# adityamwagh/SuperSLAM

Measured on AMD Instinct MI355X. Metric: stereo pairs/sec (SPx2+LG) at 1376x376, higher is better.
Workload: dtype f16; 1 GPU; configs[1]: SuperPoint x2 + select + gather + 1x LightGlue on 1376x376 stereo pairs; a step = 8 x 64 = 512 pairs per GPU resident in HBM (8 library calls of 64 pairs, different images per call), max_keypoints 600, seeded synthetic weights; pairs_per_call=64, max_keypoints=600, matches_last_call=1412, parallelism=replicated weights, pairs sharded over 1 rank(s), no data-path collective

## Files before the change

### superslam_amd/csrc/conv_pp.hip

```cpp
#include <cstdio>
#include <cstdlib>
#include <string>
#include <type_traits>
#include <vector>

#include "igemm.h"
#include "kernels.h"

#ifndef SSHIP_PP_EPI
#define SSHIP_PP_EPI -1
#endif
#ifndef SSHIP_PP_COLMAJOR
#define SSHIP_PP_COLMAJOR 1
#endif
#ifndef SSHIP_PP_EPI_LAST
#define SSHIP_PP_EPI_LAST 0
#endif
#ifndef SSHIP_PP_EPI_FUSED
#define SSHIP_PP_EPI_FUSED 0
#endif
#ifndef SSHIP_PP_TRACE_BUILD
#define SSHIP_PP_TRACE_BUILD 0
#endif
#ifndef SSHIP_PP_PRIO
#define SSHIP_PP_PRIO 2
#endif
#ifndef SSHIP_PP_NBUF
#define SSHIP_PP_NBUF 3
#endif
#ifndef SSHIP_PP_ABL
#define SSHIP_PP_ABL 0
#endif
#ifndef SSHIP_PP_ACC_PRELOAD
#define SSHIP_PP_ACC_PRELOAD 1
#endif

namespace sship {

struct PpArgs {
  const _Float16* in;
  const uint8_t* img;
  const _Float16* w1a;
  const float* b1a;
  const _Float16* wpack;
  const float* bias;
  _Float16* out;
  int B, H, W, cout;
  unsigned long long* trace;
};

constexpr int P_TH = 8, P_TW = 32, P_THH = 10, P_TWH = 34;
constexpr int P_IN_HALFS = P_THH * P_TWH * 64;
constexpr int P_W_HALFS = 36864;
constexpr int P_IN_UNITS = P_THH * P_TWH * 8;
constexpr int P_IN_IT = (P_IN_UNITS + 255) / 256;
constexpr int P_NT1A = (P_THH * P_TWH + 31) / 32;

__device__ __forceinline__ int pp_lds(int row, int col, int unit) {
  return (row * P_TWH + col) * 64 + ((unit ^ ((col >> 1) & 7)) << 3);
}

struct PpWalk { int tx, ty, b; };

template <int CIN, int CT, bool POOL, bool FUSE1A>
__global__ __launch_bounds__(512, 2) void conv3x3_pp(PpArgs p) {
  constexpr int MT = CT / 32, NCHUNK = CIN / 64;
  constexpr int EPI_MFMA = FUSE1A ? SSHIP_PP_EPI_FUSED : SSHIP_PP_EPI < 0 ? (CIN == 128 ? 2 * MT : 0) : (SSHIP_PP_EPI > 2 * MT ? 2 * MT : SSHIP_PP_EPI);
  constexpr int PIX_B = CIN * 2;
  constexpr int NBUF = SSHIP_PP_NBUF;
  static_assert(NCHUNK * 9 * 4 * MT * 512 == P_W_HALFS, "weights must fill exactly 72 KiB");
  static_assert(!FUSE1A || CIN == 64, "conv1a fusion feeds a 64-channel layer");
  extern __shared__ __attribute__((aligned(16))) char smem[];
  _Float16* s_w = reinterpret_cast<_Float16*>(smem);
  const int tid = threadIdx.x, wave = tid >> 6, lane = tid & 63, j = lane & 31, hh = lane >> 5;
  const int grp = __builtin_amdgcn_readfirstlane(wave >> 2);
  const int gw = wave & 3, gt = tid & 255;
  _Float16* my_in = s_w + P_W_HALFS + grp * P_IN_HALFS;

  const int tiles_x = (p.W + P_TW - 1) / P_TW, tiles_y = (p.H + P_TH - 1) / P_TH;
  const int ntiles = p.B * tiles_x * tiles_y;
  const int cb = blockIdx.y;
  const int t_begin = (int)((long long)blockIdx.x * ntiles / gridDim.x);
  const int t_end = (int)((long long)(blockIdx.x + 1) * ntiles / gridDim.x);
  const int n_wg = t_end - t_begin;
  if (n_wg <= 0) return;
  const int T0 = (n_wg + 1) >> 1, T1 = n_wg >> 1, T_mine = grp ? T1 : T0;

  {
    const _Float16* wsrc = p.wpack + (size_t)cb * P_W_HALFS;
    for (int u = tid; u < P_W_HALFS / 8; u += 512)
      *reinterpret_cast<uint4*>(s_w + u * 8) = *reinterpret_cast<const uint4*>(wsrc + u * 8);
  }
  float* s_bias = reinterpret_cast<float*>(s_w + P_W_HALFS + 2 * P_IN_HALFS);
  if (tid < 2 * CT) s_bias[tid] = p.bias[cb * CT + (tid % CT)];
  int boff[3][4];
#pragma unroll
  for (int kx = 0; kx < 3; ++kx)
#pragma unroll
    for (int ks = 0; ks < 4; ++ks) boff[kx][ks] = (j + kx) * 64 + (((2 * ks + hh) ^ (((j + kx) >> 1) & 7)) << 3);

  auto walk_init = [&](int t) __attribute__((always_inline)) {
    PpWalk w;
    if constexpr (SSHIP_PP_COLMAJOR != 0 && !FUSE1A) {
      w.ty = t % tiles_y;
      const int r = t / tiles_y;
      w.tx = r % tiles_x; w.b = r / tiles_x;
    } else {
      w.tx = t % tiles_x;
      const int r = t / tiles_x;
      w.ty = r % tiles_y; w.b = r / tiles_y;
    }
    return w;
  };
  auto walk_next = [&](PpWalk& w) __attribute__((always_inline)) {
    if constexpr (SSHIP_PP_COLMAJOR != 0 && !FUSE1A) {
      w.ty += 2;
      while (w.ty >= tiles_y) {
        w.ty -= tiles_y;
        if (++w.tx == tiles_x) { w.tx = 0; ++w.b; }
      }
    } else {
      w.tx += 2;
      while (w.tx >= tiles_x) {
        w.tx -= tiles_x;
        if (++w.ty == tiles_y) { w.ty = 0; ++w.b; }
      }
    }
  };
  PpWalk pw = walk_init(t_begin + grp), sw = pw, ew = pw;

  typedef unsigned u4_t __attribute__((ext_vector_type(4)));
  constexpr unsigned P_OOB = 0xfffffff0u;
  const unsigned ep_voff = POOL ? ((j & 1) ? P_OOB : (unsigned)(((j >> 1) * p.cout + hh * 8) * 2)) : (unsigned)((j * p.cout + hh * 8) * 2);
  constexpr int P_ROW_UNITS = P_TWH * 8;
  u4_t rin[FUSE1A ? 1 : 11];
  const int m_px = gt >> 3, m_part = gt & 7;
  const int r_row = gt >> 4, r_px = 32 + ((gt & 15) >> 3), r_part = gt & 7;
  const bool r_on = gt < 160;
  const unsigned voff_main = (unsigned)(m_px * PIX_B + m_part * 16);
  const unsigned voff_rem = r_on ? (unsigned)((r_row * p.W + r_px) * PIX_B + r_part * 16) : P_OOB;
  _Float16* lds_main = my_in + pp_lds(0, m_px, m_part);
  _Float16* lds_rem = my_in + pp_lds(r_on ? r_row : 0, r_px, r_part);
  const unsigned row_bytes = (unsigned)(p.W * PIX_B);
  auto prefetch_in = [&](int chunk) __attribute__((always_inline)) {
    if constexpr (!FUSE1A) {
      const int y0 = pw.ty * P_TH, x0 = pw.tx * P_TW;
      const char* img = reinterpret_cast<const char*>(p.in) + (size_t)pw.b * p.H * p.W * PIX_B - (size_t)(p.W + 1) * PIX_B;
      const __amdgpu_buffer_rsrc_t rsrc = __builtin_amdgcn_make_buffer_rsrc(const_cast<char*>(img), 0, (int)0x7ffffff0, 0x00020000);
      const unsigned soff = (unsigned)(y0 * p.W + x0) * (unsigned)PIX_B + (unsigned)chunk * 128u;
      const bool interior = y0 >= 1 && y0 + P_TH + 1 <= p.H && x0 >= 1 && x0 + P_TW + 1 <= p.W;
      if (interior) {
#pragma unroll
        for (int i = 0; i < 10; ++i) rin[i] = __builtin_amdgcn_raw_buffer_load_b128(rsrc, voff_main, soff + i * row_bytes, 0);
        rin[10] = __builtin_amdgcn_raw_buffer_load_b128(rsrc, voff_rem, soff, 0);
      } else {
        const int rlo = y0 == 0 ? 1 : 0, rhi = min(P_THH - 1, p.H - y0), clo = x0 == 0 ? 1 : 0, chi = min(P_TWH - 1, p.W - x0);
        const unsigned vm = (m_px >= clo && m_px <= chi) ? voff_main : P_OOB;
#pragma unroll
        for (int i = 0; i < 10; ++i)
          rin[i] = __builtin_amdgcn_raw_buffer_load_b128(rsrc, (i >= rlo && i <= rhi) ? vm : P_OOB, soff + i * row_bytes, 0);
        const bool r_ok = r_px >= clo && r_px <= chi && r_row >= rlo && r_row <= rhi;
        rin[10] = __builtin_amdgcn_raw_buffer_load_b128(rsrc, r_ok ? voff_rem : P_OOB, soff, 0);
      }
      if (chunk == NCHUNK - 1) walk_next(pw);
    }
  };
  auto stage_in = [&]() __attribute__((always_inline)) {
    if constexpr (!FUSE1A) {
#pragma unroll
      for (int i = 0; i < 10; ++i) *reinterpret_cast<u4_t*>(lds_main + i * (P_TWH * 64)) = rin[i];
      if (r_on) *reinterpret_cast<u4_t*>(lds_rem) = rin[10];
    }
  };
  constexpr int NT_W = 3;
  unsigned rp[FUSE1A ? NT_W : 1][3];
  int c1_pypx[FUSE1A ? NT_W : 1], c1_lds[FUSE1A ? NT_W : 1];
  const unsigned c1_selA = hh ? 0x06050402u : 0x04020100u, c1_selB = hh ? 0x0c0c0d0du : 0x0c0c0c05u;
  if constexpr (FUSE1A) {
#pragma unroll
    for (int k = 0; k < NT_W; ++k) {
      const int q = min((gw + 4 * k) * 32 + j, P_THH * P_TWH - 1);
      const int py = q / P_TWH, px = q - py * P_TWH;
      c1_pypx[k] = (py << 16) | px;
      c1_lds[k] = ((py * P_TWH + px) * 64 + hh * 4) | (((px >> 1) & 7) << 24);
    }
  }
  auto prefetch_u8 = [&]() __attribute__((always_inline)) {
    if constexpr (FUSE1A) {
      const int y0 = pw.ty * P_TH, x0 = pw.tx * P_TW;
      const uint8_t* im = p.img + (size_t)pw.b * p.H * p.W;
      walk_next(pw);
      const bool interior = y0 >= 2 && y0 + P_TH + 2 <= p.H && x0 >= 2 && x0 + P_TW + 2 + 3 <= p.W;
#pragma unroll
      for (int k = 0; k < NT_W; ++k) {
        const int py = c1_pypx[k] >> 16, px = c1_pypx[k] & 0xffff;
        if (interior) {
          const uint8_t* pp = im + (size_t)(y0 - 2 + py) * p.W + (x0 - 2 + px);
#pragma unroll
          for (int r = 0; r < 3; ++r) {
            unsigned v;
            __builtin_memcpy(&v, pp + (size_t)r * p.W, 4);
            rp[k][r] = v;
          }
        } else {
#pragma unroll
          for (int r = 0; r < 3; ++r) {
            const int cy = min(max(y0 - 2 + py + r, 0), p.H - 1), cx = min(max(x0 - 2 + px, 0), p.W - 4);
            unsigned v;
            __builtin_memcpy(&v, im + (size_t)cy * p.W + cx, 4);
            rp[k][r] = v;
          }
        }
      }
    }
  };
  h8_t a1a0, a1a1;
  if constexpr (FUSE1A) {
    a1a0 = *reinterpret_cast<const h8_t*>(p.w1a + lane * 8);
    a1a1 = *reinterpret_cast<const h8_t*>(p.w1a + 512 + lane * 8);
  }
  unsigned long long* trow = p.trace + ((size_t)(blockIdx.y * gridDim.x + blockIdx.x) * 2 + grp) * 10;
  auto stage_conv1a = [&](bool tr_stage) __attribute__((always_inline)) {
    if constexpr (FUSE1A) {
      unsigned long long ts0 = 0, ts1 = 0, ts2 = 0;
      if (SSHIP_PP_TRACE_BUILD && tr_stage) ts0 = __builtin_readcyclecounter();
      const int y0 = sw.ty * P_TH, x0 = sw.tx * P_TW;
      walk_next(sw);
      const bool interior = y0 >= 1 && y0 + P_TH + 1 <= p.H && x0 >= 1 && x0 + P_TW + 1 <= p.W;
      const bool patch_interior = y0 >= 2 && y0 + P_TH + 2 <= p.H && x0 >= 2 && x0 + P_TW + 2 + 3 <= p.W;
      h8_t bf[NT_W];
#pragma unroll
      for (int k = 0; k < NT_W; ++k) {
        if (!patch_interior) {
          const int py = c1_pypx[k] >> 16, px = c1_pypx[k] & 0xffff;
          const int gx = x0 - 2 + px;
          const int sh = gx - min(max(gx, 0), p.W - 4);
#pragma unroll
          for (int r = 0; r < 3; ++r) {
            const int gy = y0 - 2 + py + r;
            unsigned v = rp[k][r];
            v = sh < 0 ? (sh <= -4 ? 0u : v << (-8 * sh)) : (sh >= 4 ? 0u : v >> (8 * sh));
            rp[k][r] = (gy >= 0 && gy < p.H) ? v : 0u;
          }
        }
        const unsigned X = hh ? rp[k][2] : rp[k][1], Y = hh ? rp[k][1] : rp[k][0];
        const unsigned q4 = __builtin_amdgcn_perm(X, Y, c1_selA), q2 = __builtin_amdgcn_perm(X, X, c1_selB);
        auto cv8 = [](unsigned w, int byte) __attribute__((always_inline)) {
          float r;
          asm("v_mul_f32 %0, %1, %2" : "=v"(r) : "v"((float)((w >> (8 * byte)) & 0xffu)), "v"(1.0f / 255.0f));
          return (_Float16)r;
        };
        bf[k][0] = cv8(q4, 0); bf[k][1] = cv8(q4, 1); bf[k][2] = cv8(q4, 2); bf[k][3] = cv8(q4, 3);
        bf[k][4] = cv8(q2, 0); bf[k][5] = cv8(q2, 1); bf[k][6] = (_Float16)0.f; bf[k][7] = (_Float16)0.f;
      }
      if (SSHIP_PP_TRACE_BUILD && tr_stage) ts1 = __builtin_readcyclecounter();
      const f16x_t zero16 = {0.f, 0.f, 0.f, 0.f, 0.f, 0.f, 0.f, 0.f, 0.f, 0.f, 0.f, 0.f, 0.f, 0.f, 0.f, 0.f};
      f16x_t d0[NT_W], d1[NT_W];
#pragma unroll
      for (int k = 0; k < NT_W; ++k) {
        if (gw + 4 * k >= P_NT1A) continue;
        d0[k] = mfma32(a1a0, bf[k], zero16);
        d1[k] = mfma32(a1a1, bf[k], zero16);
      }
      if (SSHIP_PP_TRACE_BUILD && tr_stage) ts2 = __builtin_readcyclecounter();
#pragma unroll
      for (int k = 0; k < NT_W; ++k) {
        if (gw + 4 * k >= P_NT1A) continue;
        if ((gw + 4 * k) * 32 + j < P_THH * P_TWH) {
          bool inside = true;
          if (!interior) {
            const int gy = y0 - 1 + (c1_pypx[k] >> 16), gx = x0 - 1 + (c1_pypx[k] & 0xffff);
            inside = gy >= 0 && gy < p.H && gx >= 0 && gx < p.W;
          }
          const int base = c1_lds[k] & 0xffffff, swz = c1_lds[k] >> 24;
#pragma unroll
          for (int g = 0; g < 4; ++g) {
            const h4_t z4 = {(_Float16)0.f, (_Float16)0.f, (_Float16)0.f, (_Float16)0.f};
            h4_t o0 = __builtin_elementwise_max(to_h4(d0[k][4 * g], d0[k][4 * g + 1], d0[k][4 * g + 2], d0[k][4 * g + 3]), z4);
            h4_t o1 = __builtin_elementwise_max(to_h4(d1[k][4 * g], d1[k][4 * g + 1], d1[k][4 * g + 2], d1[k][4 * g + 3]), z4);
            if (!interior && !inside) { o0 = z4; o1 = z4; }
            const int u0 = (g ^ swz) << 3;
            *reinterpret_cast<h4_t*>(my_in + base + u0) = o0;
            *reinterpret_cast<h4_t*>(my_in + base + (u0 ^ 32)) = o1;
          }
        }
      }
      if (SSHIP_PP_TRACE_BUILD && tr_stage) { trow[6] = ts1 - ts0; trow[7] = ts2 - ts1; trow[8] = __builtin_readcyclecounter() - ts2; }
    }
  };

  f16x_t acc[MT][2];
  auto acc_init = [&]() __attribute__((always_inline)) {
#pragma unroll
    for (int m = 0; m < MT; ++m)
#pragma unroll
      for (int n = 0; n < 2; ++n)
#pragma unroll
        for (int g = 0; g < 4; ++g) {
          const float4 b4 = *reinterpret_cast<const float4*>(s_bias + n * CT + m * 32 + hh * 4 + g * 8);
          acc[m][n][4 * g + 0] = b4.x; acc[m][n][4 * g + 1] = b4.y; acc[m][n][4 * g + 2] = b4.z; acc[m][n][4 * g + 3] = b4.w;
        }
  };
  auto mfma_item = [&](auto chunk_c) __attribute__((always_inline)) {
    constexpr int chunk = decltype(chunk_c)::value;
    const _Float16* wc = s_w + chunk * (9 * 4 * MT * 512) + lane * 8;
    const _Float16* ib = my_in + (gw * 2) * P_TWH * 64;
    h8_t fa[NBUF][MT], fb[NBUF][2];
    auto load_frags = [&](int idx, int buf) __attribute__((always_inline)) {
      const int h32 = idx / 18, r18 = idx - 18 * h32, t6 = r18 / 3;
      const int ky = CIN == 128 ? r18 - 3 * t6 : (idx >> 2) / 3, kx = CIN == 128 ? t6 >> 1 : (idx >> 2) - 3 * ky;
      const int tap = ky * 3 + kx, ks = CIN == 128 ? 2 * h32 + (t6 & 1) : idx & 3;
#pragma unroll
      for (int m = 0; m < MT; ++m) fa[buf][m] = *reinterpret_cast<const h8_t*>(wc + ((tap * 4 + ks) * MT + m) * 512);
#pragma unroll
      for (int n = 0; n < 2; ++n) fb[buf][n] = *reinterpret_cast<const h8_t*>(ib + (n + ky) * P_TWH * 64 + boff[kx][ks]);
    };
    if constexpr (CIN == 64 && SSHIP_K_ROWSHARE != 0) {
      h8_t ra[3][MT], rbq[6];
      auto loads_for = [&](int t) __attribute__((always_inline)) {
        const int g = t / 3, ky = t - 3 * g, kx = g >> 2, ks = g & 3;
#pragma unroll
        for (int m = 0; m < MT; ++m) ra[t % 3][m] = *reinterpret_cast<const h8_t*>(wc + (((ky * 3 + kx) * 4 + ks) * MT + m) * 512);
        if (ky == 0) {
          rbq[(4 * g) % 6] = *reinterpret_cast<const h8_t*>(ib + boff[kx][ks]);
          rbq[(4 * g + 1) % 6] = *reinterpret_cast<const h8_t*>(ib + P_TWH * 64 + boff[kx][ks]);
        } else {
          rbq[(4 * g + ky + 1) % 6] = *reinterpret_cast<const h8_t*>(ib + (ky + 1) * P_TWH * 64 + boff[kx][ks]);
        }
      };
      loads_for(0); loads_for(1);
      if constexpr (chunk == 0 && !SSHIP_PP_ACC_PRELOAD) acc_init();
#pragma unroll
      for (int t = 0; t < 36; ++t) {
        if (t + 2 < 36 && !(SSHIP_PP_ABL & 1)) loads_for(t + 2);
        __builtin_amdgcn_sched_barrier(0);
        const int g = t / 3, ky = t - 3 * g;
#pragma unroll
        for (int n = 0; n < 2; ++n)
#pragma unroll
          for (int m = 0; m < MT; ++m) {
            if constexpr ((SSHIP_PP_ABL & 2) != 0) asm volatile("" :: "v"(ra[t % 3][m]), "v"(rbq[(4 * g + ky + n) % 6]));
            else acc[m][n] = mfma32(ra[t % 3][m], rbq[(4 * g + ky + n) % 6], acc[m][n]);
          }
        __builtin_amdgcn_sched_barrier(0);
      }
      return;
    }
#pragma unroll
    for (int i = 0; i < NBUF - 1; ++i) load_frags(i, i);
    if constexpr (chunk == 0 && !SSHIP_PP_ACC_PRELOAD) acc_init();
#pragma unroll
    for (int idx = 0; idx < 36; ++idx) {
      if (idx + NBUF - 1 < 36 && !(SSHIP_PP_ABL & 1)) load_frags(idx + NBUF - 1, (idx + NBUF - 1) % NBUF);
      __builtin_amdgcn_sched_barrier(0);
#pragma unroll
      for (int n = 0; n < 2; ++n)
#pragma unroll
        for (int m = 0; m < MT; ++m) {
          if constexpr ((SSHIP_PP_ABL & 2) != 0) asm volatile("" :: "v"(fa[idx % NBUF][m]), "v"(fb[idx % NBUF][n]));
          else acc[m][n] = mfma32(fa[idx % NBUF][m], fb[idx % NBUF][n], acc[m][n]);
        }
      __builtin_amdgcn_sched_barrier(0);
    }
  };
  auto epilogue = [&](int u_lo, int u_hi) __attribute__((always_inline)) {
    const int y0 = ew.ty * P_TH, x0 = ew.tx * P_TW, b = ew.b;
    if (u_hi == 2 * MT) walk_next(ew);
    const int yb = y0 + __builtin_amdgcn_readfirstlane(gw) * 2;
    const h2_t z2 = {(_Float16)0.f, (_Float16)0.f};
    auto relu2 = [&](float lo, float hi) __attribute__((always_inline)) -> unsigned {
      h2_t v = {(_Float16)lo, (_Float16)hi};
      v = __builtin_elementwise_max(v, z2);
      return *reinterpret_cast<const unsigned*>(&v);
    };
    auto pack2 = [](float lo, float hi) __attribute__((always_inline)) -> unsigned {
      const h2_t v = {(_Float16)lo, (_Float16)hi};
      return *reinterpret_cast<const unsigned*>(&v);
    };
    const int Ho = POOL ? p.H >> 1 : p.H, Wo = POOL ? p.W >> 1 : p.W;
    const __amdgpu_buffer_rsrc_t ro = __builtin_amdgcn_make_buffer_rsrc(
        reinterpret_cast<char*>(p.out) + (size_t)b * Ho * Wo * p.cout * 2, 0, (int)0x7ffffff0, 0x00020000);
    const int xo0 = POOL ? x0 >> 1 : x0;
    unsigned voff = ep_voff;
    if (xo0 + (POOL ? P_TW / 2 : P_TW) > Wo)
      voff = (xo0 + (POOL ? j >> 1 : j)) < Wo ? ep_voff : P_OOB;
    auto store_pair = [&](int row_off, int m, int g, unsigned a0, unsigned a1, unsigned b0, unsigned b1) __attribute__((always_inline)) {
      const auto r0 = __builtin_amdgcn_permlane32_swap(a0, b0, false, false);
      const auto r1 = __builtin_amdgcn_permlane32_swap(a1, b1, false, false);
      int so = (row_off + cb * CT + m * 32 + g * 8) * 2;
      asm volatile("" : "+s"(so));
      typedef unsigned st4_t __attribute__((ext_vector_type(4)));
      if constexpr ((SSHIP_PP_ABL & 4) != 0) { asm volatile("" :: "v"(r0[0]), "v"(r1[0]), "v"(r0[1]), "v"(r1[1])); return; }
      __builtin_amdgcn_raw_buffer_store_b128(st4_t{r0[0], r1[0], r0[1], r1[1]}, ro, voff, so, 0);
    };
    if constexpr (!POOL) {
      const int x = x0 + j;
#pragma unroll
      for (int n = 0; n < 2; ++n) {
        const int y = yb + n;
        const bool ok = y < p.H && x < p.W;
        _Float16* pix = p.out + ((size_t)(b * p.H + y) * p.W + x) * p.cout + cb * CT;
#pragma unroll
        for (int m = 0; m < MT; ++m)
#pragma unroll
          for (int g = 0; g < 4; g += 2) {
            if (2 * m + g / 2 < u_lo || 2 * m + g / 2 >= u_hi) continue;
            const f16x_t& a = acc[m][n];
            const auto r0 = __builtin_amdgcn_permlane32_swap(relu2(a[4 * g + 0], a[4 * g + 1]), relu2(a[4 * g + 4], a[4 * g + 5]), false, false);
            const auto r1 = __builtin_amdgcn_permlane32_swap(relu2(a[4 * g + 2], a[4 * g + 3]), relu2(a[4 * g + 6], a[4 * g + 7]), false, false);
            if constexpr ((SSHIP_PP_ABL & 4) != 0) { asm volatile("" :: "v"(r0[0]), "v"(r1[0]), "v"(r0[1]), "v"(r1[1])); continue; }
            if (ok) *reinterpret_cast<uint4*>(pix + m * 32 + (g + hh) * 8) = make_uint4(r0[0], r1[0], r0[1], r1[1]);
          }
      }
    } else {
      const int yo = yb >> 1;
      if (yo >= Ho) voff = P_OOB;
      const int pix = (yo * Wo + xo0) * p.cout;
      auto pool1 = [&](int m, int r) __attribute__((always_inline)) -> float {
        const float tt = fmaxf(fmaxf(acc[m][0][r], acc[m][1][r]), 0.f);
        const float nb = __int_as_float(__builtin_amdgcn_update_dpp(0, __float_as_int(tt), 0xB1, 0xF, 0xF, false));
        return fmaxf(tt, nb);
      };
#pragma unroll
      for (int m = 0; m < MT; ++m)
#pragma unroll
        for (int g = 0; g < 4; g += 2) {
          if (2 * m + g / 2 < u_lo || 2 * m + g / 2 >= u_hi) continue;
          store_pair(pix, m, g, pack2(pool1(m, 4 * g + 0), pool1(m, 4 * g + 1)), pack2(pool1(m, 4 * g + 2), pool1(m, 4 * g + 3)),
                     pack2(pool1(m, 4 * g + 4), pool1(m, 4 * g + 5)), pack2(pool1(m, 4 * g + 6), pool1(m, 4 * g + 7)));
        }
    }
  };

  const bool tr_lane = SSHIP_PP_TRACE_BUILD && p.trace && gw == 0 && lane == 0;
  unsigned long long t0 = 0, t1 = 0;
  auto data_role = [&](bool do_epi, bool do_stage, bool do_prefetch, int pf_chunk, bool init_acc, bool tr) __attribute__((always_inline)) {
    if (SSHIP_PP_PRIO) __builtin_amdgcn_s_setprio(SSHIP_PP_PRIO);
    if (tr) t0 = __builtin_readcyclecounter();
    if (!SSHIP_PP_EPI_LAST && do_epi && EPI_MFMA < 2 * MT) epilogue(EPI_MFMA, 2 * MT);
    if (tr) { t1 = __builtin_readcyclecounter(); trow[0] = t1 - t0; t0 = t1; }
    if (do_stage) { if constexpr (FUSE1A) stage_conv1a(tr); else stage_in(); }
    if (tr) { t1 = __builtin_readcyclecounter(); trow[1] = t1 - t0; t0 = t1; }
    if (do_prefetch) { if constexpr (FUSE1A) prefetch_u8(); else prefetch_in(pf_chunk); }
    if (SSHIP_PP_EPI_LAST && do_epi && EPI_MFMA < 2 * MT) epilogue(EPI_MFMA, 2 * MT);
    if (SSHIP_PP_ACC_PRELOAD && init_acc) acc_init();
    if (tr) { t1 = __builtin_readcyclecounter(); trow[2] = t1 - t0; t0 = t1; }
    __syncthreads();
    if (tr) trow[4] = __builtin_readcyclecounter() - t0;
    if (SSHIP_PP_PRIO) __builtin_amdgcn_s_setprio(0);
  };
  auto mfma_role = [&](auto chunk_c, bool tr) __attribute__((always_inline)) {
    constexpr int chunk = decltype(chunk_c)::value;
    if (tr) t0 = __builtin_readcyclecounter();
    mfma_item(chunk_c);
    if constexpr (chunk == NCHUNK - 1 && EPI_MFMA > 0) epilogue(0, EPI_MFMA);
    if (tr) { t1 = __builtin_readcyclecounter(); trow[3] = t1 - t0; t0 = t1; }
    __syncthreads();
    if (tr) trow[5] = __builtin_readcyclecounter() - t0;
  };
  const std::integral_constant<int, 0> c0{};
  const std::integral_constant<int, NCHUNK - 1> c_last{};
  const int nbar_mine = grp + 1 + 2 * NCHUNK * T_mine, nbar_all = max(1 + 2 * NCHUNK * T0, 2 + 2 * NCHUNK * T1);
  if (T_mine > 0) { if constexpr (FUSE1A) prefetch_u8(); else prefetch_in(0); }
  __syncthreads();
  if (grp == 1) __syncthreads();
  data_role(false, T_mine > 0, NCHUNK > 1 ? T_mine > 0 : T_mine > 1, NCHUNK > 1 ? 1 : 0, T_mine > 0, false);
#pragma unroll 1
  for (int it = 0; it < T_mine; ++it) {
    const bool more = it + 1 < T_mine, tr = tr_lane && it == 2;
    if constexpr (NCHUNK == 1) {
      mfma_role(c0, tr);
      data_role(true, more, it + 2 < T_mine, 0, more, tr);
    } else {
      mfma_role(c0, tr);
      data_role(false, true, more, 0, false, tr);
      mfma_role(c_last, false);
      data_role(true, more, more, 1, more, false);
    }
  }
#pragma unroll 1
  for (int k = nbar_mine; k < nbar_all; ++k) __syncthreads();
}

template <int CIN, int CT, bool POOL, bool FUSE1A>
static hipError_t launch_pp(const PpArgs& a_in, hipStream_t s) {
  PpArgs a = a_in;
  constexpr size_t smem = (size_t)(2 * P_IN_HALFS + P_W_HALFS) * 2 + 128 * 4;
  static_assert(smem <= 163840, "LDS budget");
  auto kern = conv3x3_pp<CIN, CT, POOL, FUSE1A>;
  static const hipError_t attr_rc = hipFuncSetAttribute(reinterpret_cast<const void*>(kern), hipFuncAttributeMaxDynamicSharedMemorySize, (int)smem);
  if (attr_rc != hipSuccess) return attr_rc;
  const int ncb = a.cout / CT;
  const int ntiles = a.B * ((a.W + P_TW - 1) / P_TW) * ((a.H + P_TH - 1) / P_TH);
  int gx = cu_count() / ncb;
  if (gx < 1) gx = 1;
  if (gx * 2 > ntiles) gx = (ntiles + 1) / 2;
  if (gx < 1) gx = 1;
  static const bool trace_on = SSHIP_PP_TRACE_BUILD && dev_env("SSHIP_PP_TRACE") != nullptr;
  static unsigned long long* tbuf = nullptr;
  if (trace_on) {
    if (!tbuf) (void)hipMalloc(&tbuf, 4096 * 2 * 10 * 8);
    (void)hipMemsetAsync(tbuf, 0, 4096 * 2 * 10 * 8, s);
    a.trace = tbuf;
  }
  hipLaunchKernelGGL(kern, dim3(gx, ncb), dim3(512), smem, s, a);
  if (trace_on) {
    std::vector<unsigned long long> h(4096 * 2 * 10);
    (void)hipStreamSynchronize(s);
    (void)hipMemcpy(h.data(), tbuf, h.size() * 8, hipMemcpyDeviceToHost);
    double sum[10] = {0}; long cnt = 0;
    for (int i = 0; i < gx * ncb * 2; ++i) {
      if (!h[i * 10 + 3]) continue;
      for (int k = 0; k < 10; ++k) sum[k] += (double)h[i * 10 + k];
      ++cnt;
    }
    if (cnt) fprintf(stderr, "[pp trace cin=%d ct=%d pool=%d fuse=%d] epilogue=%.0f stage=%.0f prefetch=%.0f | mfma=%.0f | barrier wait after data=%.0f after mfma=%.0f (clk, %ld groups)\n",
                     CIN, CT, (int)POOL, (int)FUSE1A, sum[0] / cnt, sum[1] / cnt, sum[2] / cnt, sum[3] / cnt, sum[4] / cnt, sum[5] / cnt, cnt);
    if (cnt && sum[6] > 0) fprintf(stderr, "[pp trace   conv1a staging] convert=%.0f mfma issue=%.0f relu+lds writes=%.0f clk\n", sum[6] / cnt, sum[7] / cnt, sum[8] / cnt);
  }
  return hipGetLastError();
}

hipError_t sp_conv3x3_pp(const ConvW& w, const _Float16* in, _Float16* out, int B, int H, int W, bool pool, hipStream_t s) {
  if ((size_t)H * W * w.cin * 2 >= 0x7f000000ull) return hipErrorInvalidValue;
  PpArgs a{};
  a.in = in; a.wpack = w.w; a.bias = w.bias; a.out = out; a.B = B; a.H = H; a.W = W; a.cout = w.cout;
  static const bool dma64 = [] { const char* e = dev_env("SUPERSLAM_HIP_CONV64"); return e && std::string(e) == "dma"; }();
  if (w.cin == 64 && w.w_q && dma64 && sp_conv3x3_pp128_fits(B, H, W, 64)) return sp_conv3x3_pp128(w, in, out, B, H, W, pool, s);
  if (w.cin == 64 && w.ct == 64) return pool ? launch_pp<64, 64, true, false>(a, s) : launch_pp<64, 64, false, false>(a, s);
  static const std::string c128 = [] { const char* e = dev_env("SUPERSLAM_HIP_CONV128"); return std::string(e ? e : ""); }();
  static const bool ct32 = c128 == "ct32";
  const int tiles16 = B * ((W + 31) / 32) * ((H + 15) / 16);
  const bool few_tiles = c128.empty() && w.ct == 32 && w.w && (tiles16 + 1) / 2 * (w.cout / 64) < cu_count();
  if (w.cin == 128 && w.w_q && !ct32 && !few_tiles && sp_conv3x3_pp128_fits(B, H, W, 128)) return sp_conv3x3_pp128(w, in, out, B, H, W, pool, s);
  if (w.cin == 128 && w.ct == 32) return pool ? launch_pp<128, 32, true, false>(a, s) : launch_pp<128, 32, false, false>(a, s);
  return hipErrorInvalidValue;
}

hipError_t sp_conv1ab_pp(const ConvW& w1b, const _Float16* w1a_frag, const float* b1a, const uint8_t* img, _Float16* out,
                         int B, int H, int W, hipStream_t s) {
  PpArgs a{};
  a.img = img; a.w1a = w1a_frag; a.b1a = b1a; a.wpack = w1b.w; a.bias = w1b.bias; a.out = out;
  a.B = B; a.H = H; a.W = W; a.cout = w1b.cout;
  if (w1b.cin != 64 || w1b.ct != 64) return hipErrorInvalidValue;
  return launch_pp<64, 64, true, true>(a, s);
}

}
```

Baseline: 5688 pairs/s.

## Keep conv1b weights in registers and repartition waves in fused conv1a+conv1b kernel

For the fused conv1a+conv1b (64-channel, pooled) kernel, each wave now holds its slice of the 3x3 weights in 36 VGPR fragments instead of reading them from a 72 KiB LDS copy. Waves split the two M-tiles by gw&1 and cover four output rows each, streaming input rows from LDS with a 6-deep rotating buffer. To free registers, the conv1a per-lane coordinate tables and weights move to LDS, and there is a new pooled epilogue path. This removes the LDS weight traffic and shrinks LDS use, but raises VGPR pressure and adds LDS lookups in the staging code.

After: 5693 pairs/s, median of 2. No clear change (+0.1%).

```diff
diff --git a/superslam_amd/csrc/conv_pp.hip b/superslam_amd/csrc/conv_pp.hip
--- a/superslam_amd/csrc/conv_pp.hip
+++ b/superslam_amd/csrc/conv_pp.hip
@@ -33,6 +33,9 @@
 #endif
 #ifndef SSHIP_PP_ACC_PRELOAD
 #define SSHIP_PP_ACC_PRELOAD 1
+#endif
+#ifndef SSHIP_PP_WREG
+#define SSHIP_PP_WREG 1
 #endif
 
 namespace sship {
@@ -55,6 +58,7 @@
 constexpr int P_IN_UNITS = P_THH * P_TWH * 8;
 constexpr int P_IN_IT = (P_IN_UNITS + 255) / 256;
 constexpr int P_NT1A = (P_THH * P_TWH + 31) / 32;
+constexpr bool pp_wreg(int cin, bool fuse1a) { return cin == 64 && fuse1a && SSHIP_PP_WREG != 0 && SSHIP_K_ROWSHARE != 0; }
 
 __device__ __forceinline__ int pp_lds(int row, int col, int unit) {
   return (row * P_TWH + col) * 64 + ((unit ^ ((col >> 1) & 7)) << 3);
@@ -67,15 +71,21 @@
   constexpr int MT = CT / 32, NCHUNK = CIN / 64;
   constexpr int EPI_MFMA = FUSE1A ? SSHIP_PP_EPI_FUSED : SSHIP_PP_EPI < 0 ? (CIN == 128 ? 2 * MT : 0) : (SSHIP_PP_EPI > 2 * MT ? 2 * MT : SSHIP_PP_EPI);
   constexpr int PIX_B = CIN * 2;
+  constexpr bool WREG = pp_wreg(CIN, FUSE1A);
+  constexpr int MW = WREG ? 1 : MT, NB = WREG ? 4 : 2;
+  constexpr int W_HALFS = WREG ? 0 : P_W_HALFS;
   constexpr int NBUF = SSHIP_PP_NBUF;
   static_assert(NCHUNK * 9 * 4 * MT * 512 == P_W_HALFS, "weights must fill exactly 72 KiB");
   static_assert(!FUSE1A || CIN == 64, "conv1a fusion feeds a 64-channel layer");
+  static_assert(!WREG || MT == 2, "register-resident weights: waves gw & 1 split the two M-tiles of a 64-channel cout tile");
   extern __shared__ __attribute__((aligned(16))) char smem[];
   _Float16* s_w = reinterpret_cast<_Float16*>(smem);
   const int tid = threadIdx.x, wave = tid >> 6, lane = tid & 63, j = lane & 31, hh = lane >> 5;
+  const int wave_s = __builtin_amdgcn_readfirstlane(wave);
   const int grp = __builtin_amdgcn_readfirstlane(wave >> 2);
   const int gw = wave & 3, gt = tid & 255;
-  _Float16* my_in = s_w + P_W_HALFS + grp * P_IN_HALFS;
+  _Float16* my_in = s_w + W_HALFS + grp * P_IN_HALFS;
+  const int mw = __builtin_amdgcn_readfirstlane(gw & 1), row0 = __builtin_amdgcn_readfirstlane(gw >> 1) * 4;
 
   const int tiles_x = (p.W + P_TW - 1) / P_TW, tiles_y = (p.H + P_TH - 1) / P_TH;
   const int ntiles = p.B * tiles_x * tiles_y;
@@ -86,13 +96,25 @@
   if (n_wg <= 0) return;
   const int T0 = (n_wg + 1) >> 1, T1 = n_wg >> 1, T_mine = grp ? T1 : T0;
 
-  {
+  h8_t wr[WREG ? 36 : 1];
+  if constexpr (WREG) {
+    const _Float16* wsrc = p.wpack + (size_t)cb * P_W_HALFS + mw * 512 + lane * 8;
+#pragma unroll
+    for (int i = 0; i < 36; ++i) wr[i] = *reinterpret_cast<const h8_t*>(wsrc + i * (MT * 512));
+  } else {
     const _Float16* wsrc = p.wpack + (size_t)cb * P_W_HALFS;
     for (int u = tid; u < P_W_HALFS / 8; u += 512)
       *reinterpret_cast<uint4*>(s_w + u * 8) = *reinterpret_cast<const uint4*>(wsrc + u * 8);
   }
-  float* s_bias = reinterpret_cast<float*>(s_w + P_W_HALFS + 2 * P_IN_HALFS);
-  if (tid < 2 * CT) s_bias[tid] = p.bias[cb * CT + (tid % CT)];
+  float* s_bias = reinterpret_cast<float*>(s_w + W_HALFS + 2 * P_IN_HALFS);
+  if (tid < NB * CT) s_bias[tid] = p.bias[cb * CT + (tid % CT)];
+  _Float16* s_a1a = reinterpret_cast<_Float16*>(s_bias + NB * CT);
+  int2* s_c1 = reinterpret_cast<int2*>(s_a1a + 1024) + tid;
+  auto lane_now = [&]() __attribute__((always_inline)) -> int {
+    int l = lane;
+    if constexpr (WREG) asm volatile("" : "+v"(l));
+    return l;
+  };
   int boff[3][4];
 #pragma unroll
   for (int kx = 0; kx < 3; ++kx)
@@ -174,17 +196,24 @@
   };
   constexpr int NT_W = 3;
   unsigned rp[FUSE1A ? NT_W : 1][3];
-  int c1_pypx[FUSE1A ? NT_W : 1], c1_lds[FUSE1A ? NT_W : 1];
+  int c1_pypx[FUSE1A && !WREG ? NT_W : 1], c1_lds[FUSE1A && !WREG ? NT_W : 1];
   const unsigned c1_selA = hh ? 0x06050402u : 0x04020100u, c1_selB = hh ? 0x0c0c0d0du : 0x0c0c0c05u;
   if constexpr (FUSE1A) {
 #pragma unroll
     for (int k = 0; k < NT_W; ++k) {
       const int q = min((gw + 4 * k) * 32 + j, P_THH * P_TWH - 1);
       const int py = q / P_TWH, px = q - py * P_TWH;
-      c1_pypx[k] = (py << 16) | px;
-      c1_lds[k] = ((py * P_TWH + px) * 64 + hh * 4) | (((px >> 1) & 7) << 24);
-    }
+      const int pypx = (py << 16) | px, ldsw = ((py * P_TWH + px) * 64 + hh * 4) | (((px >> 1) & 7) << 24);
+      if constexpr (WREG) s_c1[k * 512] = make_int2(pypx, ldsw);
+      else { c1_pypx[k] = pypx; c1_lds[k] = ldsw; }
+    }
+    if constexpr (WREG)
+      if (tid < 128) *reinterpret_cast<uint4*>(s_a1a + tid * 8) = *reinterpret_cast<const uint4*>(p.w1a + tid * 8);
   }
+  auto c1_get = [&](int k) __attribute__((always_inline)) -> int2 {
+    if constexpr (WREG) return (s_c1 - tid)[k * 512 + wave_s * 64 + lane_now()];
+    else return make_int2(c1_pypx[k], c1_lds[k]);
+  };
   auto prefetch_u8 = [&]() __attribute__((always_inline)) {
     if constexpr (FUSE1A) {
       const int y0 = pw.ty * P_TH, x0 = pw.tx * P_TW;
@@ -193,7 +222,7 @@
       const bool interior = y0 >= 2 && y0 + P_TH + 2 <= p.H && x0 >= 2 && x0 + P_TW + 2 + 3 <= p.W;
 #pragma unroll
       for (int k = 0; k < NT_W; ++k) {
-        const int py = c1_pypx[k] >> 16, px = c1_pypx[k] & 0xffff;
+        const int pypx = c1_get(k).x, py = pypx >> 16, px = pypx & 0xffff;
         if (interior) {
           const uint8_t* pp = im + (size_t)(y0 - 2 + py) * p.W + (x0 - 2 + px);
 #pragma unroll
@@ -215,7 +244,7 @@
     }
   };
   h8_t a1a0, a1a1;
-  if constexpr (FUSE1A) {
+  if constexpr (FUSE1A && !WREG) {
     a1a0 = *reinterpret_cast<const h8_t*>(p.w1a + lane * 8);
     a1a1 = *reinterpret_cast<const h8_t*>(p.w1a + 512 + lane * 8);
   }
@@ -229,10 +258,12 @@
       const bool interior = y0 >= 1 && y0 + P_TH + 1 <= p.H && x0 >= 1 && x0 + P_TW + 1 <= p.W;
       const bool patch_interior = y0 >= 2 && y0 + P_TH + 2 <= p.H && x0 >= 2 && x0 + P_TW + 2 + 3 <= p.W;
       h8_t bf[NT_W];
+      const int ln = lane_now();
+      const unsigned selA = WREG ? ((ln >> 5) ? 0x06050402u : 0x04020100u) : c1_selA, selB = WREG ? ((ln >> 5) ? 0x0c0c0d0du : 0x0c0c0c05u) : c1_selB;
 #pragma unroll
       for (int k = 0; k < NT_W; ++k) {
         if (!patch_interior) {
-          const int py = c1_pypx[k] >> 16, px = c1_pypx[k] & 0xffff;
+          const int pypx = c1_get(k).x, py = pypx >> 16, px = pypx & 0xffff;
           const int gx = x0 - 2 + px;
           const int sh = gx - min(max(gx, 0), p.W - 4);
 #pragma unroll
@@ -244,7 +275,7 @@
           }
         }
         const unsigned X = hh ? rp[k][2] : rp[k][1], Y = hh ? rp[k][1] : rp[k][0];
-        const unsigned q4 = __builtin_amdgcn_perm(X, Y, c1_selA), q2 = __builtin_amdgcn_perm(X, X, c1_selB);
+        const unsigned q4 = __builtin_amdgcn_perm(X, Y, selA), q2 = __builtin_amdgcn_perm(X, X, selB);
         auto cv8 = [](unsigned w, int byte) __attribute__((always_inline)) {
           float r;
           asm("v_mul_f32 %0, %1, %2" : "=v"(r) : "v"((float)((w >> (8 * byte)) & 0xffu)), "v"(1.0f / 255.0f));
@@ -255,49 +286,73 @@
       }
       if (SSHIP_PP_TRACE_BUILD && tr_stage) ts1 = __builtin_readcyclecounter();
       const f16x_t zero16 = {0.f, 0.f, 0.f, 0.f, 0.f, 0.f, 0.f, 0.f, 0.f, 0.f, 0.f, 0.f, 0.f, 0.f, 0.f, 0.f};
-      f16x_t d0[NT_W], d1[NT_W];
-#pragma unroll
-      for (int k = 0; k < NT_W; ++k) {
-        if (gw + 4 * k >= P_NT1A) continue;
-        d0[k] = mfma32(a1a0, bf[k], zero16);
-        d1[k] = mfma32(a1a1, bf[k], zero16);
-      }
-      if (SSHIP_PP_TRACE_BUILD && tr_stage) ts2 = __builtin_readcyclecounter();
-#pragma unroll
-      for (int k = 0; k < NT_W; ++k) {
-        if (gw + 4 * k >= P_NT1A) continue;
-        if ((gw + 4 * k) * 32 + j < P_THH * P_TWH) {
+      auto write_out = [&](int k, const f16x_t& d, int mt) __attribute__((always_inline)) {
+        if ((gw + 4 * k) * 32 + (WREG ? ln & 31 : j) < P_THH * P_TWH) {
+          const int2 c1k = c1_get(k);
           bool inside = true;
           if (!interior) {
-            const int gy = y0 - 1 + (c1_pypx[k] >> 16), gx = x0 - 1 + (c1_pypx[k] & 0xffff);
+            const int gy = y0 - 1 + (c1k.x >> 16), gx = x0 - 1 + (c1k.x & 0xffff);
             inside = gy >= 0 && gy < p.H && gx >= 0 && gx < p.W;
           }
-          const int base = c1_lds[k] & 0xffffff, swz = c1_lds[k] >> 24;
+          const int base = c1k.y & 0xffffff, swz = c1k.y >> 24;
 #pragma unroll
           for (int g = 0; g < 4; ++g) {
             const h4_t z4 = {(_Float16)0.f, (_Float16)0.f, (_Float16)0.f, (_Float16)0.f};
-            h4_t o0 = __builtin_elementwise_max(to_h4(d0[k][4 * g], d0[k][4 * g + 1], d0[k][4 * g + 2], d0[k][4 * g + 3]), z4);
-            h4_t o1 = __builtin_elementwise_max(to_h4(d1[k][4 * g], d1[k][4 * g + 1], d1[k][4 * g + 2], d1[k][4 * g + 3]), z4);
-            if (!interior && !inside) { o0 = z4; o1 = z4; }
+            h4_t o = __builtin_elementwise_max(to_h4(d[4 * g], d[4 * g + 1], d[4 * g + 2], d[4 * g + 3]), z4);
+            if (!interior && !inside) o = z4;
             const int u0 = (g ^ swz) << 3;
-            *reinterpret_cast<h4_t*>(my_in + base + u0) = o0;
-            *reinterpret_cast<h4_t*>(my_in + base + (u0 ^ 32)) = o1;
-          }
+            *reinterpret_cast<h4_t*>(my_in + base + (mt ? u0 ^ 32 : u0)) = o;
+          }
+        }
+      };
+      if constexpr (WREG) {
+#pragma unroll
+        for (int mt = 0; mt < 2; ++mt) {
+          f16x_t d[NT_W];
+          const h8_t a1 = *reinterpret_cast<const h8_t*>(s_a1a + mt * 512 + ln * 8);
+#pragma unroll
+          for (int k = 0; k < NT_W; ++k) {
+            if (gw + 4 * k >= P_NT1A) continue;
+            d[k] = mfma32(a1, bf[k], zero16);
+          }
+          if (SSHIP_PP_TRACE_BUILD && tr_stage && mt == 1) ts2 = __builtin_readcyclecounter();
+#pragma unroll
+          for (int k = 0; k < NT_W; ++k) {
+            if (gw + 4 * k >= P_NT1A) continue;
+            write_out(k, d[k], mt);
+          }
+          __builtin_amdgcn_sched_barrier(0);
+        }
+      } else {
+        f16x_t d0[NT_W], d1[NT_W];
+#pragma unroll
+        for (int k = 0; k < NT_W; ++k) {
+          if (gw + 4 * k >= P_NT1A) continue;
+          d0[k] = mfma32(a1a0, bf[k], zero16);
+          d1[k] = mfma32(a1a1, bf[k], zero16);
+        }
+        if (SSHIP_PP_TRACE_BUILD && tr_stage) ts2 = __builtin_readcyclecounter();
+#pragma unroll
+        for (int k = 0; k < NT_W; ++k) {
+          if (gw + 4 * k >= P_NT1A) continue;
+          write_out(k, d0[k], 0);
+          write_out(k, d1[k], 1);
         }
       }
       if (SSHIP_PP_TRACE_BUILD && tr_stage) { trow[6] = ts1 - ts0; trow[7] = ts2 - ts1; trow[8] = __builtin_readcyclecounter() - ts2; }
     }
   };
 
-  f16x_t acc[MT][2];
+  f16x_t acc[MW][NB];
   auto acc_init = [&]() __attribute__((always_inline)) {
-#pragma unroll
-    for (int m = 0; m < MT; ++m)
-#pragma unroll
-      for (int n = 0; n < 2; ++n)
+    const int hh_i = WREG ? lane_now() >> 5 : hh;
+#pragma unroll
+    for (int m = 0; m < MW; ++m)
+#pragma unroll
+      for (int n = 0; n < NB; ++n)
 #pragma unroll
         for (int g = 0; g < 4; ++g) {
-          const float4 b4 = *reinterpret_cast<const float4*>(s_bias + n * CT + m * 32 + hh * 4 + g * 8);
+          const float4 b4 = *reinterpret_cast<const float4*>(s_bias + n * CT + (WREG ? mw : m) * 32 + hh_i * 4 + g * 8);
           acc[m][n][4 * g + 0] = b4.x; acc[m][n][4 * g + 1] = b4.y; acc[m][n][4 * g + 2] = b4.z; acc[m][n][4 * g + 3] = b4.w;
         }
   };
@@ -315,6 +370,39 @@
 #pragma unroll
       for (int n = 0; n < 2; ++n) fb[buf][n] = *reinterpret_cast<const h8_t*>(ib + (n + ky) * P_TWH * 64 + boff[kx][ks]);
     };
+    if constexpr (WREG) {
+      const _Float16* ib4 = my_in + row0 * P_TWH * 64;
+      int kxor[4] = {0, 16, 32, 48};
+      asm volatile("" : "+s"(kxor[1]), "+s"(kxor[2]), "+s"(kxor[3]));
+      const int lm = lane_now(), jm = lm & 31, hm = lm >> 5;
+      int kb[3];
+#pragma unroll
+      for (int kx = 0; kx < 3; ++kx) kb[kx] = (jm + kx) * 64 + ((hm ^ (((jm + kx) >> 1) & 7)) << 3);
+      h8_t rb[6];
+      auto load_row = [&](int q) __attribute__((always_inline)) {
+        const int g = q / 6, r = q - 6 * g, kx = g >> 2, ks = g & 3;
+        rb[q % 6] = *reinterpret_cast<const h8_t*>(ib4 + r * P_TWH * 64 + (ks ? kb[kx] ^ kxor[ks] : kb[kx]));
+      };
+#pragma unroll
+      for (int q = 0; q < 5; ++q) load_row(q);
+      if constexpr ((SSHIP_PP_ABL & 1) != 0) rb[5] = rb[0];
+      if constexpr (chunk == 0 && !SSHIP_PP_ACC_PRELOAD) acc_init();
+#pragma unroll
+      for (int q = 0; q < 72; ++q) {
+        if (q + 5 < 72 && !(SSHIP_PP_ABL & 1)) load_row(q + 5);
+        __builtin_amdgcn_sched_barrier(0);
+        const int g = q / 6, r = q - 6 * g, kx = g >> 2, ks = g & 3;
+#pragma unroll
+        for (int ky = 0; ky < 3; ++ky) {
+          const int n = r - ky;
+          if (n < 0 || n > 3) continue;
+          if constexpr ((SSHIP_PP_ABL & 2) != 0) asm volatile("" :: "v"(wr[(ky * 3 + kx) * 4 + ks]), "v"(rb[q % 6]));
+          else acc[0][n] = mfma32(wr[(ky * 3 + kx) * 4 + ks], rb[q % 6], acc[0][n]);
+        }
+        __builtin_amdgcn_sched_barrier(0);
+      }
+      return;
+    }
     if constexpr (CIN == 64 && SSHIP_K_ROWSHARE != 0) {
       h8_t ra[3][MT], rbq[6];
       auto loads_for = [&](int t) __attribute__((always_inline)) {
@@ -366,7 +454,7 @@
   auto epilogue = [&](int u_lo, int u_hi) __attribute__((always_inline)) {
     const int y0 = ew.ty * P_TH, x0 = ew.tx * P_TW, b = ew.b;
     if (u_hi == 2 * MT) walk_next(ew);
-    const int yb = y0 + __builtin_amdgcn_readfirstlane(gw) * 2;
+    const int yb = y0 + (WREG ? row0 : __builtin_amdgcn_readfirstlane(gw) * 2);
     const h2_t z2 = {(_Float16)0.f, (_Float16)0.f};
     auto relu2 = [&](float lo, float hi) __attribute__((always_inline)) -> unsigned {
       h2_t v = {(_Float16)lo, (_Float16)hi};
@@ -382,9 +470,13 @@
         reinterpret_cast<char*>(p.out) + (size_t)b * Ho * Wo * p.cout * 2, 0, (int)0x7ffffff0, 0x00020000);
     const int xo0 = POOL ? x0 >> 1 : x0;
     unsigned voff = ep_voff;
+    if constexpr (WREG) {
+      const int l = lane_now(), jl = l & 31, hl = l >> 5;
+      voff = POOL ? ((jl & 1) ? P_OOB : (unsigned)(((jl >> 1) * p.cout + hl * 8) * 2)) : (unsigned)((jl * p.cout + hl * 8) * 2);
+    }
     if (xo0 + (POOL ? P_TW / 2 : P_TW) > Wo)
-      voff = (xo0 + (POOL ? j >> 1 : j)) < Wo ? ep_voff : P_OOB;
-    auto store_pair = [&](int row_off, int m, int g, unsigned a0, unsigned a1, unsigned b0, unsigned b1) __attribute__((always_inline)) {
+      voff = (xo0 + (POOL ? j >> 1 : j)) < Wo ? voff : P_OOB;
+    auto store_pair = [&](unsigned voff, int row_off, int m, int g, unsigned a0, unsigned a1, unsigned b0, unsigned b1) __attribute__((always_inline)) {
       const auto r0 = __builtin_amdgcn_permlane32_swap(a0, b0, false, false);
       const auto r1 = __builtin_amdgcn_permlane32_swap(a1, b1, false, false);
       int so = (row_off + cb * CT + m * 32 + g * 8) * 2;
@@ -393,7 +485,28 @@
       if constexpr ((SSHIP_PP_ABL & 4) != 0) { asm volatile("" :: "v"(r0[0]), "v"(r1[0]), "v"(r0[1]), "v"(r1[1])); return; }
       __builtin_amdgcn_raw_buffer_store_b128(st4_t{r0[0], r1[0], r0[1], r1[1]}, ro, voff, so, 0);
     };
-    if constexpr (!POOL) {
+    if constexpr (WREG) {
+      static_assert(!WREG || POOL, "the register-weight block serves the pooled conv1a + conv1b kernel");
+      {
+#pragma unroll
+        for (int q = 0; q < 2; ++q) {
+          const int yo = (yb >> 1) + q;
+          const unsigned vo = yo >= Ho ? P_OOB : voff;
+          const int pix = (yo * Wo + xo0) * p.cout;
+          auto pool1 = [&](int r) __attribute__((always_inline)) -> float {
+            const float tt = fmaxf(fmaxf(acc[0][2 * q][r], acc[0][2 * q + 1][r]), 0.f);
+            const float nb = __int_as_float(__builtin_amdgcn_update_dpp(0, __float_as_int(tt), 0xB1, 0xF, 0xF, false));
+            return fmaxf(tt, nb);
+          };
+#pragma unroll
+          for (int g = 0; g < 4; g += 2) {
+            if (2 * q + g / 2 < u_lo || 2 * q + g / 2 >= u_hi) continue;
+            store_pair(vo, pix, mw, g, pack2(pool1(4 * g + 0), pool1(4 * g + 1)), pack2(pool1(4 * g + 2), pool1(4 * g + 3)),
+                       pack2(pool1(4 * g + 4), pool1(4 * g + 5)), pack2(pool1(4 * g + 6), pool1(4 * g + 7)));
+          }
+        }
+      }
+    } else if constexpr (!POOL) {
       const int x = x0 + j;
 #pragma unroll
       for (int n = 0; n < 2; ++n) {
@@ -426,7 +539,7 @@
 #pragma unroll
         for (int g = 0; g < 4; g += 2) {
           if (2 * m + g / 2 < u_lo || 2 * m + g / 2 >= u_hi) continue;
-          store_pair(pix, m, g, pack2(pool1(m, 4 * g + 0), pool1(m, 4 * g + 1)), pack2(pool1(m, 4 * g + 2), pool1(m, 4 * g + 3)),
+          store_pair(voff, pix, m, g, pack2(pool1(m, 4 * g + 0), pool1(m, 4 * g + 1)), pack2(pool1(m, 4 * g + 2), pool1(m, 4 * g + 3)),
                      pack2(pool1(m, 4 * g + 4), pool1(m, 4 * g + 5)), pack2(pool1(m, 4 * g + 6), pool1(m, 4 * g + 7)));
         }
     }
@@ -439,8 +552,10 @@
     if (tr) t0 = __builtin_readcyclecounter();
     if (!SSHIP_PP_EPI_LAST && do_epi && EPI_MFMA < 2 * MT) epilogue(EPI_MFMA, 2 * MT);
     if (tr) { t1 = __builtin_readcyclecounter(); trow[0] = t1 - t0; t0 = t1; }
+    if constexpr (WREG) __builtin_amdgcn_sched_barrier(0);
     if (do_stage) { if constexpr (FUSE1A) stage_conv1a(tr); else stage_in(); }
     if (tr) { t1 = __builtin_readcyclecounter(); trow[1] = t1 - t0; t0 = t1; }
+    if constexpr (WREG) __builtin_amdgcn_sched_barrier(0);
     if (do_prefetch) { if constexpr (FUSE1A) prefetch_u8(); else prefetch_in(pf_chunk); }
     if (SSHIP_PP_EPI_LAST && do_epi && EPI_MFMA < 2 * MT) epilogue(EPI_MFMA, 2 * MT);
     if (SSHIP_PP_ACC_PRELOAD && init_acc) acc_init();
@@ -470,7 +585,7 @@
     const bool more = it + 1 < T_mine, tr = tr_lane && it == 2;
     if constexpr (NCHUNK == 1) {
       mfma_role(c0, tr);
-      data_role(true, more, it + 2 < T_mine, 0, more, tr);
+      data_role(true, more, it + 2 < T_mine, 0, WREG ? true : more, tr);
     } else {
       mfma_role(c0, tr);
       data_role(false, true, more, 0, false, tr);
@@ -485,7 +600,8 @@
 template <int CIN, int CT, bool POOL, bool FUSE1A>
 static hipError_t launch_pp(const PpArgs& a_in, hipStream_t s) {
   PpArgs a = a_in;
-  constexpr size_t smem = (size_t)(2 * P_IN_HALFS + P_W_HALFS) * 2 + 128 * 4;
+  constexpr size_t smem = pp_wreg(CIN, FUSE1A) ? (size_t)2 * P_IN_HALFS * 2 + 256 * 4 + 1024 * 2 + 3 * 512 * 8
+                                                : (size_t)(2 * P_IN_HALFS + P_W_HALFS) * 2 + 128 * 4;
   static_assert(smem <= 163840, "LDS budget");
   auto kern = conv3x3_pp<CIN, CT, POOL, FUSE1A>;
   static const hipError_t attr_rc = hipFuncSetAttribute(reinterpret_cast<const void*>(kern), hipFuncAttributeMaxDynamicSharedMemorySize, (int)smem);
```
